# cavelandiah/BBMap

Hardware: AMD Instinct MI355X
Metric: aligned_reads_per_sec (higher is better)
Workload: dtype int32

## Files before the change

bbmap_amd/csrc/msa_common.h:

```cpp
#pragma once
#include <hip/hip_runtime.h>
#include <stdint.h>
#include "bbmap_amd.h"

namespace bbmsa {

constexpr int kScoreOffset = 11;
constexpr int kTimeMask = 0x7FF;
constexpr int kScoreMask = (int)0xFFFFF800;
constexpr int kMaxTime = 2047;

#define BBMSA_PT(x) ((x) * 2048)
constexpr int P_MATCH = BBMSA_PT(70), P_MATCH2 = BBMSA_PT(100);
constexpr int P_SUB = BBMSA_PT(-127), P_SUBR = BBMSA_PT(-147), P_SUB2 = BBMSA_PT(-51), P_SUB3 = BBMSA_PT(-25);
constexpr int P_INS = BBMSA_PT(-395), P_INS2 = BBMSA_PT(-39), P_INS3 = BBMSA_PT(-23), P_INS4 = BBMSA_PT(-8);
constexpr int P_DEL = BBMSA_PT(-472), P_DEL2 = BBMSA_PT(-33), P_DEL3 = BBMSA_PT(-9), P_DEL4 = BBMSA_PT(-1),
              P_DEL5 = BBMSA_PT(-1);
constexpr int P_DEL_REF_N = BBMSA_PT(-10), P_GAP = BBMSA_PT(-2);
constexpr int kBadOff = (-(((1 << 20) - 1) - 2000) - 1) * 2048;
constexpr int kMinOffScore = (-(((1 << 20) - 1) - 2000)) * 2048;
constexpr int kNegInf = -(1 << 30);
constexpr int kGapLen = 128;

constexpr int kTableLen = 3072;
__host__ __device__ inline int lds_table_ints(int tableLen) { return 2 * tableLen + 320; }

__host__ __device__ inline int lds_job_ints(int fastCols, int tmpBytes) { return (fastCols + 2) + ((fastCols + 2 + 3) >> 2) + ((tmpBytes + 3) >> 2); }

__host__ __device__ inline int calc_del_off(int len) {
    if (len <= 0) return 0;
    int s = P_DEL;
    if (len > 80) { s += ((len - 80 + 3) / 4) * P_DEL5; len = 80; }
    if (len > 20) { s += (len - 20) * P_DEL4; len = 20; }
    if (len > 5) { s += (len - 5) * P_DEL3; len = 5; }
    if (len > 1) s += (len - 1) * P_DEL2;
    return s;
}
__host__ __device__ inline int calc_ins_cum_off(int len) {
    if (len <= 0) return 0;
    long long s = P_INS;
    int n = len;
    if (n > 20) { s += (long long)(n - 20) * P_INS4; n = 20; }
    if (n > 5) { s += (long long)(n - 5) * P_INS3; n = 5; }
    if (n > 1) s += (long long)(n - 1) * P_INS2;
    return s < kMinOffScore ? kMinOffScore : (int)s;
}

__host__ __device__ inline bool fully_defined(int b) {
    const int u = b & ~32;
    return b < 128 && (u == 'A' || u == 'C' || u == 'G' || u == 'T' || u == 'U');
}

struct Scheme11ts {
    static constexpr int OFF = kScoreOffset, TMASK = kTimeMask, SMASK = kScoreMask, MAXT = kMaxTime;
    static constexpr int MATCH = P_MATCH, MATCH2 = P_MATCH2, SUB = P_SUB, SUBR = P_SUBR, SUB2 = P_SUB2, SUB3 = P_SUB3;
    static constexpr int INS = P_INS, INS2 = P_INS2, INS3 = P_INS3, INS4 = P_INS4;
    static constexpr int DEL = P_DEL, DEL2 = P_DEL2, DEL3 = P_DEL3, DEL4 = P_DEL4, DEL5 = P_DEL5;
    static constexpr int DEL_REF_N = P_DEL_REF_N, GAP = P_GAP;
    static constexpr int BAR_I1 = 2, BAR_D1 = 3;
    static constexpr int BADOFF = kBadOff;
    __host__ __device__ static inline int del_off(int len) { return calc_del_off(len); }
    __host__ __device__ static inline int ins_cum_off(int len) { return calc_ins_cum_off(len); }
    __host__ __device__ static inline int col0(int row) { return calc_ins_cum_off(row); }
};
struct Scheme9PacBio {
    static constexpr int OFF = 9, TMASK = 0x1FF, SMASK = (int)0xFFFFFE00, MAXT = 511;
#define BBMSA_PB(x) ((x) * 512)
    static constexpr int MATCH = BBMSA_PB(90), MATCH2 = BBMSA_PB(100);
    static constexpr int SUB = BBMSA_PB(-137), SUBR = BBMSA_PB(-157), SUB2 = BBMSA_PB(-49), SUB3 = BBMSA_PB(-25);
    static constexpr int INS = BBMSA_PB(-205), INS2 = BBMSA_PB(-42), INS3 = BBMSA_PB(-23), INS4 = BBMSA_PB(-8);
    static constexpr int DEL = BBMSA_PB(-292), DEL2 = BBMSA_PB(-37), DEL3 = BBMSA_PB(-17), DEL4 = BBMSA_PB(-2), DEL5 = BBMSA_PB(-1);
    static constexpr int DEL_REF_N = BBMSA_PB(-10), GAP = BBMSA_PB(-2);
    static constexpr int BAR_I1 = 1, BAR_D1 = 1;
    static constexpr int BADOFF = (-(((1 << 22) - 1) - 2000) - 1) * 512;
#undef BBMSA_PB
    __host__ __device__ static inline int del_off(int len) {
        if (len <= 0) return 0;
        int s = DEL;
        if (len > 80) { s += ((len - 80 + 3) / 4) * DEL5; len = 80; }
        if (len > 20) { s += (len - 20) * DEL4; len = 20; }
// ... 99 lines not shown
```

bbmap_amd/csrc/msa_fill_fast.hip:

```cpp
#include "msa_common.h"
#include "msa_cell.h"

namespace bbmsa {

__device__ __forceinline__ int lane_up(int x, int fill) {
    return __builtin_amdgcn_update_dpp(fill, x, 0x138, 0xf, 0xf, false);
}

__device__ __forceinline__ int clamp_time(int t) { return t > kMaxTime ? kMaxTime - 3 : t; }

__device__ __forceinline__ int del_extend(int streak) {
    int c = (streak & 3) == 0 ? P_DEL5 : 0;
    c = streak < 80 ? P_DEL4 : c;
    c = streak < 20 ? P_DEL3 : c;
    c = streak < 5 ? P_DEL2 : c;
    c = streak == 0 ? P_DEL : c;
    return c;
}
__device__ __forceinline__ int ins_extend(int streak) {
    int c = P_INS4;
    c = streak < 20 ? P_INS3 : c;
    c = streak < 5 ? P_INS2 : c;
    c = streak == 0 ? P_INS : c;
    return c;
}
__device__ __forceinline__ int sub_extend(int streak) {
    int c = P_SUB3;
    c = streak < 5 ? P_SUB2 : c;
    c = streak == 0 ? P_SUB : c;
    return c;
}

__device__ __forceinline__ unsigned load_coherent(const unsigned *p) {
    return __hip_atomic_load(p, __ATOMIC_RELAXED, __HIP_MEMORY_SCOPE_AGENT);
}

#ifndef BBMSA_MIN_WAVES
#define BBMSA_MIN_WAVES(R) ((R) <= 5 ? 4 : ((R) <= 7 ? 2 : 1))
#endif

template <int R, bool BANDED, bool MAT = false>
__global__ __launch_bounds__(256, BBMSA_MIN_WAVES(R)) void msa_fill_fast_kernel(const FillParams p) {
    extern __shared__ int lds[];
    int *delC = lds;
    const int TL = p.tableLen;
    int *insC = lds + TL;
    int *delExt = lds + 2 * TL;
    int *insExt = delExt + 128;
    int4 *mTab = reinterpret_cast<int4 *>(delExt + 192);
    LdsPen pen; pen.delC = delC; pen.insC = insC; pen.delExt = delExt; pen.insExt = insExt; pen.mTab = mTab;
    for (int i = threadIdx.x; i < TL; i += blockDim.x) {
        delC[i] = calc_del_off(i);
        insC[i] = calc_ins_cum_off(i);
    }
    for (int i = threadIdx.x; i < 128; i += blockDim.x) delExt[i] = del_extend(i);
    if (threadIdx.x < 32) insExt[threadIdx.x] = ins_extend(threadIdx.x);
    if (threadIdx.x < 32) {
        const int st = threadIdx.x & 7, mt = (threadIdx.x >> 3) & 1, pv = threadIdx.x >> 4;
        int4 e;
        if (mt) { e.x = pv ? P_MATCH2 : P_MATCH; e.y = P_MATCH; e.z = P_MATCH2; }
        else { e.x = pv ? (st <= 1 ? P_SUBR : P_SUB) : sub_extend(min(st, 5)); e.y = P_SUB; e.z = P_SUB3; }
        e.w = 0;
        mTab[threadIdx.x] = e;
    }
    __syncthreads();

    if (p.priority == 3) __builtin_amdgcn_s_setprio(3);
    else if (p.priority == 2) __builtin_amdgcn_s_setprio(2);
    else if (p.priority == 1) __builtin_amdgcn_s_setprio(1);
    const int lane = threadIdx.x & 63;
    const int wave = threadIdx.x >> 6;
    const int G = p.lanesPerJob;
    const int gl = lane & (G - 1);
    const int sub = lane / G;
    const int jobsPerWave = 64 / G;
    const int groupBase = sub * G;

    const int perJobLds = lds_job_ints(p.fastCols, p.tmpBytes);
    int *myLds = lds + lds_table_ints(TL) + (wave * jobsPerWave + sub) * perJobLds;
    int *colHl = myLds;
    uint8_t *colRef = reinterpret_cast<uint8_t *>(myLds + (p.fastCols + 2));
    uint8_t *tmp = reinterpret_cast<uint8_t *>(myLds + (p.fastCols + 2) + ((p.fastCols + 2 + 3) >> 2));

    const long long slot = ((long long)blockIdx.x * (blockDim.x >> 6) + wave) * jobsPerWave + sub;
    unsigned *dir = p.dirbuf + slot * p.dir_slot_dwords;

    const long long total = p.list ? (long long)load_coherent(p.list_count) : job_count(p.njobs, p.njobs_dev);
    for (;;) {
        unsigned base = 0;
        if (lane == 0) base = atomicAdd(p.queue, (unsigned)jobsPerWave);
        base = __builtin_amdgcn_readfirstlane(base);
        if ((long long)base >= total) break;
        const long long q = (long long)base + sub;
        const bool valid = q < total;
        const long long j = (p.list && valid) ? (long long)p.list[q] : q;

        bbmsa_job jb;
        if (valid) jb = p.jobs[j];
        else { jb.read_off = 0; jb.ref_off = 0; jb.read_len = 0; jb.ref_len = 0; jb.refStartLoc = 0; jb.refEndLoc = -1; jb.minScore = 0; jb.flags = 0; }
        const int rows = jb.read_len;
        int a = jb.refStartLoc, b = jb.refEndLoc;
        const int mode = jb.flags & BBMSA_MODE_MASK;
        if (jb.flags & BBMSA_CLAMP_WINDOW) {
            a = max(0, a);
            b = min(jb.ref_len - 1, b);
            if (b - a >= p.maxColumns) b = min(jb.ref_len - 1, a + p.maxColumns - 1);
        }
        const int columns = b - a + 1;
        const bool shapeOK = valid && rows >= 1 && columns >= 1 && rows <= p.maxRows && columns <= p.maxColumns;

        int halfband = 0;
        if (!(p.bandwidth < 1 && p.bandwidthRatio <= 0.0f)) {
            const int bwA = p.bandwidth < 1 ? 9999999 : p.bandwidth;
            const int bwB = p.bandwidthRatio <= 0.0f ? 9999999 : 8 + (int)__fmul_rn((float)rows, p.bandwidthRatio);
            halfband = max(min(bwA, bwB), columns - rows + 8) / 2;
        }
        int minScore = jb.minScore;
        bool limited;
        if (mode == BBMSA_FILL_UNLIMITED_RAW) limited = false;
        else if (mode == BBMSA_FILL_LIMITED_RAW) limited = true;
        else {
            if (minScore < 1 || (columns + rows < 90) ||
                ((halfband < 1 || halfband * 3 > columns) && (columns > rows + min(170, rows + 20)))) limited = false;
            else { limited = true; minScore -= 120; }
        }
        const bool fits = rows <= G * R && columns <= p.fastCols && columns >= rows - 2;
        const bool needGeneric = shapeOK && !fits;
        const bool run = shapeOK && !needGeneric;
        const bool banded = limited && halfband > 0;
        int bandViolation = 0;

        if (gl == 0 && valid) {
            if (!shapeOK) {
                bbmsa_result r;
                for (int i = 0; i < 5; i++) r.result[i] = 0;
                r.status = BBMSA_ST_BAD_SHAPE; r.iterations = 0;
                for (int i = 0; i < 8; i++) r.score[i] = 0;
                r.score_len = 0; r.match_len = 0; r.fill_kind = 0; r.columns = columns;
// ... 41 lines not shown
                cst[k] = c;
                laneSum += c;
            }
            int inc = laneSum;
            for (int d = 1; d < G; d <<= 1) {
                const int o = __shfl_down(inc, d, 64);
                if (gl + d < G) inc += o;
            }
            int suffix = inc - laneSum;
#pragma unroll
            for (int k = R - 1; k >= 0; k--) {
                suffix += cst[k];
                vlim[k] = limited ? max(minScoreOff - suffix, floorv) : kNegInf;
            }
            if (MAT && run && limited) {
                int *vout = p.limits + p.limits_off[j];
#pragma unroll
                for (int k = 0; k < R; k++) if (r0 + k < rows) vout[r0 + k] = vlim[k];
                if (gl == 0) {
                    vout[rows] = minScoreOff;
                    const int c0 = fully_defined(call1[0]) ? ((rows > 1 && fully_defined(idxByte[0])) ? P_MATCH2 : P_MATCH) : 0;
                    vout[0] = rows > 1 ? max(vlim[0] - c0, floorv) : max(minScoreOff - c0, floorv);
                }
            }
        }

        if (run) {
            for (int c = gl + 1; c <= columns; c += G) colRef[c] = rf[c - 1];
        }
        __builtin_amdgcn_fence(__ATOMIC_ACQ_REL, "wavefront");
        __builtin_amdgcn_wave_barrier();
        if (run && gl == 0) {
            int h = minScoreOff;
            bool prevDef = false;
            for (int i = columns - 1; i >= 0; i--) {
                colHl[i + 1] = (limited ? h : kNegInf) + 2048;
                const int cb = colRef[i + 1];
                const bool def = fully_defined(cb);
                const int cost = def ? (prevDef ? P_MATCH2 : P_MATCH) : ((prevDef && cb == '-') ? P_DEL : 0);
                h = max(h - cost, floorv);
                prevDef = def;
                if (MAT && limited) p.limits[p.limits_off[j] + rows + 1 + i + 1] = colHl[i + 1] - 2048;
            }
            if (MAT && limited) p.limits[p.limits_off[j] + rows + 1] = h;
        }
        __builtin_amdgcn_fence(__ATOMIC_ACQ_REL, "wavefront");
        __builtin_amdgcn_wave_barrier();

        const int nl = (rows + R - 1) / R;
        int steps = run ? columns + nl - 1 : 0;
        for (int d = 32; d >= 1; d >>= 1) steps = max(steps, __shfl_xor(steps, d, 64));

        int pM[R], pD[R], pI[R];
        int minGood[R], maxGood[R];
        int vlimP[R];
        int delForce[R];
        int insHiForce[R];
        unsigned dacc[R];
        int mPrev[R];
#pragma unroll
        for (int k = 0; k < R; k++) {
            const int row = r0 + k;
            const int c0v = insC[row];
            pM[k] = c0v; pD[k] = c0v; pI[k] = c0v;
            minGood[k] = -1; maxGood[k] = -2; dacc[k] = 0;
            vlimP[k] = rowValid[k] ? vlim[k] + 2048 : (1 << 30);
            mPrev[k] = (call1[k] == '!') ? 8 : 0;
            delForce[k] = (row < 3 || row > rows - 3) ? INT_MAX : INT_MIN;
            insHiForce[k] = (row > rows - 2) ? INT_MAX : INT_MIN;
        }
        const bool rowOne = (r0 == 1);
        const bool notLimited = !limited;
        const bool groupLead = (gl == 0);
        const int floorP = floorv + 2048;
        int svM = insC[r0 - 1], svD = svM, svI = svM;
        int lastRef = '!';
        const int lastSlot = (max(rows, 1) - 1) % R;
        const bool ownerLaneFlag = gl == (max(rows, 1) - 1) / R;
        int bestM = 0, bestD = 0, bestI = 0, bestMc = -1, bestDc = -1, bestIc = -1;

        for (int t = 1; t <= steps; t++) {
            const int c = t - gl;
            if (c >= 1 && run) {
            const bool inRange = c <= columns;
            const int cc = min(c, columns);
            const int hlP = colHl[cc], ref1 = colRef[cc];
            const int ref0 = c < 2 ? '!' : lastRef;
            const bool gap = ref1 == '-';
            const bool refN = ref1 == 'N';
            const int refPen = refN ? P_DEL_REF_N : (gap ? P_GAP : 0);
            const int insNeededBase = (columns - c) + 1;
            const bool cGt1 = c > 1;
            const int cLtLastForce = (c < columns - 1) ? INT_MAX : INT_MIN;
            const unsigned sh = (unsigned)(t & 7) * 4u;

            int upM = lane_up(pM[R - 1], 0);
            int upD = lane_up(pD[R - 1], 0);
            int upI = lane_up(pI[R - 1], 0);
            int upMin = lane_up(minGood[R - 1], 1);
            upM = groupLead ? 0 : upM; upD = groupLead ? 0 : upD; upI = groupLead ? 0 : upI;
            upMin = groupLead ? 1 : upMin;
            int upMaxG = 0;
            if (BANDED) {
                upMaxG = lane_up(maxGood[R - 1], 0);
                upMaxG = groupLead ? min(columns, 2 * halfband) : upMaxG;
            }
            int dgM = svM, dgD = svD, dgI = svI;
            svM = upM; svD = upD; svI = upI;
            bool started = upMin >= 0;
            int pm8 = ((call0First == ref0) & (ref0 != 'N')) ? 8 : 0;

#pragma unroll
            for (int k = 0; k < R; k++) {
                const int row = r0 + k;
                bool act = inRange & (started | notLimited);
                if (BANDED) act = act && (!banded || (c >= row - halfband && c <= upMaxG + 1));
                CellIn ci_;
                ci_.row = row; ci_.c = c; ci_.rows = rows; ci_.insNeededBase = insNeededBase;
                ci_.cl1 = call1[k]; ci_.ref1 = ref1; ci_.refN = refN; ci_.gap = gap; ci_.match = (call1[k] == ref1) & !refN; ci_.act = act;
                ci_.refPen = refPen; ci_.limitP = max(vlimP[k], hlP); ci_.floorP = floorP; ci_.subfloor = subfloor;
                ci_.dgM = dgM; ci_.dgD = dgD; ci_.dgI = dgI; ci_.lM = pM[k]; ci_.lD = pD[k]; ci_.upM = upM; ci_.upI = upI;
                ci_.delForce = delForce[k];
                ci_.insForce = (k == 0) ? ((rowOne && cGt1) ? INT_MAX : min(insHiForce[k], cLtLastForce)) : min(insHiForce[k], cLtLastForce);
                ci_.pm8 = pm8;
                const CellOut co = cell_update<Scheme11ts, false>(pen, ci_);
                const int nM = co.nM, nD = co.nD, nI = co.nI;
                const bool goodM = co.goodM, goodD = co.goodD, goodI = co.goodI;
                const int mb8 = co.mb8;
                if (MAT) {
                    if (inRange & rowValid[k]) {
                        int *cellp = planeM + (long long)(row - 1) * planeW + (c - 1);
                        const int sM = co.pruneM ? subfloor : (goodM ? nM : (subfloor | clamp_cell_time<Scheme11ts>(co.timeM)));
                        const int sD = co.pruneD ? subfloor : (goodD ? nD : (subfloor | clamp_cell_time<Scheme11ts>(co.timeD)));
                        const int sI = co.pruneI ? subfloor : (goodI ? nI : (subfloor | clamp_cell_time<Scheme11ts>(co.timeI)));
                        cellp[0] = sM; cellp[planeInts] = sD; cellp[2 * planeInts] = sI;
                    }
                }
                dacc[k] |= co.nib << sh;

                const bool good = goodM | goodD | goodI;
                if (BANDED) {
                    if (good && banded && minGood[k] >= 0 && c - maxGood[k] >= 3 && row < rows) bandViolation = 1;
                }
                minGood[k] = (good & (minGood[k] < 0)) ? c : minGood[k];
                maxGood[k] = good ? c : maxGood[k];
                dgM = pM[k]; dgD = pD[k]; dgI = pI[k];
                pM[k] = nM; pD[k] = nD; pI[k] = nI;
                upM = nM; upI = nI;
                started = minGood[k] >= 0;
                if (BANDED) upMaxG = maxGood[k];
                pm8 = mPrev[k];
                mPrev[k] = mb8;
            }
            lastRef = ref1;

            {
                int lm = pM[0], ld = pD[0], li = pI[0];
#pragma unroll
                for (int k = 1; k < R; k++) {
                    lm = (lastSlot == k) ? pM[k] : lm; ld = (lastSlot == k) ? pD[k] : ld; li = (lastSlot == k) ? pI[k] : li;
                }
                const bool track = ownerLaneFlag & inRange;
                const bool um = track & ((bestMc < 0) | ((lm & kScoreMask) > (bestM & kScoreMask)));
                const bool ud = track & ((bestDc < 0) | ((ld & kScoreMask) > (bestD & kScoreMask)));
                const bool ui = track & ((bestIc < 0) | ((li & kScoreMask) > (bestI & kScoreMask)));
                bestM = um ? lm : bestM; bestMc = um ? c : bestMc;
                bestD = ud ? ld : bestD; bestDc = ud ? c : bestDc;
                bestI = ui ? li : bestI; bestIc = ui ? c : bestIc;
            }
            }

            if ((t & 7) == 7) {
                const long long o = (long long)(t >> 3) * R * G + gl;
#pragma unroll
                for (int k = 0; k < R; k++) { dir[o + (long long)k * G] = dacc[k]; dacc[k] = 0; }
            }
        }
        if ((steps & 7) != 7) {
            const long long o = (long long)(steps >> 3) * R * G + gl;
#pragma unroll
            for (int k = 0; k < R; k++) dir[o + (long long)k * G] = dacc[k];
        }

        int firstNoEnter = INT_MAX;
        int lastColStart = 1, lastHasGood = 0;
        long long itersAll[R];
        {
            int pMin = lane_up(minGood[R - 1], 1), pMax = lane_up(maxGood[R - 1], columns);
            if (gl == 0) { pMin = 1; pMax = columns; }
#pragma unroll
            for (int k = 0; k < R; k++) {
                const int row = r0 + k;
                itersAll[k] = 0;
                if (rowValid[k]) {
                    const int hasGood = minGood[k] >= 0;
                    const int colStart = banded ? max(pMin, row - halfband) : pMin;
                    const int colStop = banded ? min(pMax, row + 2 * halfband - 1) : pMax;
                    const bool enter = pMin >= 0 && colStart >= 0 && colStop >= colStart;
                    if (!enter && firstNoEnter == INT_MAX) firstNoEnter = row;
                    const int endc = banded ? min(columns, colStop + 1)
                                            : min(columns, max(colStop, hasGood ? maxGood[k] : -2) + 1);
                    itersAll[k] = (long long)(endc - colStart + 1);
                    if (row == rows) { lastColStart = colStart; lastHasGood = hasGood; }
                }
                pMin = minGood[k]; pMax = maxGood[k];
            }
        }
        int groupNoEnter = firstNoEnter;
        for (int d = 1; d < G; d <<= 1) groupNoEnter = min(groupNoEnter, __shfl_xor(groupNoEnter, d, 64));
        long long iters = 0;
#pragma unroll
        for (int k = 0; k < R; k++) if (rowValid[k] && r0 + k < groupNoEnter) iters += itersAll[k];
        for (int d = 1; d < G; d <<= 1) iters += __shfl_xor(iters, d, 64);
        if (!limited) iters = (long long)rows * columns;
        for (int d = 1; d < G; d <<= 1) bandViolation |= __shfl_xor(bandViolation, d, 64);

        const int ownerLane = groupBase + (max(rows, 1) - 1) / R;
        int bScore, bCol, bState, bPacked;
        {
            int s = bestMc >= 0 ? (bestM & kScoreMask) : INT_MIN, cbest = bestMc, st = 0, pk = bestM;
            if (bestDc >= 0 && (bestD & kScoreMask) > s) { s = bestD & kScoreMask; cbest = bestDc; st = 1; pk = bestD; }
            if (bestIc >= 0 && (bestI & kScoreMask) > s) { s = bestI & kScoreMask; cbest = bestIc; st = 2; pk = bestI; }
            bScore = __shfl(s, ownerLane, 64);
            bCol = __shfl(cbest, ownerLane, 64);
            bState = __shfl(st, ownerLane, 64);
            bPacked = __shfl(pk, ownerLane, 64);
            lastColStart = __shfl(lastColStart, ownerLane, 64);
            lastHasGood = __shfl(lastHasGood, ownerLane, 64);
        }

        int res0 = rows, res1, res2, res3, res4 = 0;
        bool fillNull = false;
        if (!limited) {
            res1 = bCol; res2 = bState; res3 = bScore >> kScoreOffset;
        } else if (groupNoEnter <= rows) {
            res1 = 1; res2 = 0; res3 = kBadOff; res4 = 1; fillNull = true;
        } else if (!lastHasGood) {
            res1 = max(1, lastColStart - 1); res2 = 0; res3 = subfloor; res4 = 1; fillNull = true;
        } else if (bScore < minScoreOff) {
            res1 = bCol; res2 = bState; res3 = bScore; res4 = 1; fillNull = true;
        } else {
            res1 = bCol; res2 = bState; res3 = bScore >> kScoreOffset;
        }

        const bool wantScore = run && !fillNull && !bandViolation && (jb.flags & BBMSA_DO_SCORE);
        const bool wantTrace = run && !fillNull && !bandViolation && (jb.flags & BBMSA_DO_TRACEBACK) && p.match != nullptr;
        int sc[8] = {0, 0, 0, 0, 0, 0, 0, 0};
        int scoreLen = 0, matchLen = 0;

        asm volatile("s_waitcnt vmcnt(0)" ::: "memory");
        __builtin_amdgcn_wave_barrier();

        if (__any(wantScore || wantTrace)) {
            const bool walk = wantScore || wantTrace;
            int row = walk ? rows : 0, col = walk ? res1 : 0, state = res2;
            int n = 0, gapSyms = 0, stateTime = 0;
            while (__any(row > 0 && col > 0)) {
                const bool go = row > 0 && col > 0;
                if (go && state == 0) {
                    const int rr = row - gl, cq = col - gl;
                    const bool inside = rr >= 1 && cq >= 1;
                    unsigned nibv = 0;
                    if (inside) {
                        const int ol = (rr - 1) / R, ok = (rr - 1) - ol * R, ot = cq + ol;
                        const unsigned dw = load_coherent(dir + ((long long)(ot >> 3) * R + ok) * G + ol);
                        nibv = (dw >> ((ot & 7) * 4)) & 15u;
                    }
                    const bool brk = !inside || (nibv & 3u) != 0u;
                    unsigned long long bal = __ballot(brk);
                    unsigned long long mine = (G == 64) ? bal : ((bal >> groupBase) & ((1ull << G) - 1ull));
                    const int fb = mine ? __builtin_ctzll(mine) : G;
                    const int fbInside = __shfl((int)inside, groupBase + min(fb, G - 1), 64);
                    const int fbPrev = __shfl((int)(nibv & 3u), groupBase + min(fb, G - 1), 64);
                    const int consumed = (fb < G && fbInside) ? fb + 1 : fb;
                    if (wantTrace && gl < consumed) {
                        const int cb = rd[rr - 1], rb = colRef[cq];
                        tmp[n + gl] = (cb == rb) ? 'm' : ((!fully_defined(cb) || !fully_defined(rb)) ? 'N' : 'S');
                    }
                    stateTime += fb;
// ... 112 lines not shown
```

bbmap_amd/csrc/msa_host.hip:

```cpp
#include <hip/hip_runtime.h>

#include <cstdio>
#include <cstdlib>
#include <cstring>
#include <new>

#include "msa_common.h"

int bbmsa_align_impl(bbmsa_ctx *c, void *stream_, int64_t n_jobs, const uint32_t *n_jobs_dev, const bbmsa_job *jobs,
                     const uint8_t *reads, const uint8_t *refs, bbmsa_result *results, uint8_t *match, int32_t match_stride);

namespace bbmsa {
struct StripParams {
    const bbmsa_job *jobs; const uint8_t *reads; const uint8_t *refs; bbmsa_result *results; uint8_t *match;
    long long njobs; const unsigned int *njobs_dev; unsigned int *queue; unsigned int *dirbuf;
    long long dir_slot_dwords, dir_strip_dwords; int *boundary; uint8_t *tmpbuf; int *slow_list; unsigned int *slow_count;
    int match_stride; int maxRows, maxColumns; int bandwidth; float bandwidthRatio;
    int pipeK, pipeSlots; int *pipeBoundary; int *pipeSync; int pipeSpinLimit;
};
int strip_rows_per_lane();
const void *strip_kernel_pacbio();
const void *strip_kernel_pacbio_pipelined();
int strip_pipe_sync_ints(int K);
const void *fast_kernel_for(int R, bool banded);
// ... 18 lines not shown
    const int t = threadIdx.x;
    s[t] = hist[t];
    __syncthreads();
    for (int d = 1; d < WIDTH_BUCKETS; d <<= 1) { const unsigned v = t >= d ? s[t - d] : 0u; __syncthreads(); s[t] += v; __syncthreads(); }
    hist[t] = s[t] - hist[t];
    if (t == 0) *listCount = n;
}
__global__ void width_scatter_kernel(const bbmsa_job *jobs, long long n, int maxColumns, unsigned *cursor, int *list) {
    const long long i = (long long)blockIdx.x * blockDim.x + threadIdx.x;
    if (i < n) list[atomicAdd(&cursor[job_width_bucket(jobs[i], maxColumns)], 1u)] = (int)i;
}
}

static thread_local char g_err[512] = "";

static int fail(int code, const char *fmt, const char *detail = "") {
    snprintf(g_err, sizeof g_err, fmt, detail);
    return code;
}
#define HIP_TRY(expr)                                                                      \
    do {                                                                                   \
        hipError_t e_ = (expr);                                                            \
        if (e_ != hipSuccess) {                                                            \
            snprintf(g_err, sizeof g_err, "%s failed: %s", #expr, hipGetErrorString(e_));  \
            return BBMAP_E_HIP;                                                            \
        }                                                                                  \
    } while (0)

#include "msa_ctx.h"

extern "C" const char *bbmap_last_error(void) { return g_err; }
void bbmap_set_error(const char *msg) { snprintf(g_err, sizeof g_err, "%s", msg); }
extern "C" int bbmap_abi_version(void) { return BBMAP_AMD_ABI_VERSION; }

static int env_int(const char *name, int dflt) {
    const char *v = getenv(name);
    return (v && *v) ? atoi(v) : dflt;
}

static int setup_wide_pass(bbmsa_ctx *c) {
    if (c->wideBlocks > 0) return BBMAP_OK;
    c->wideR = (c->cfg.maxRows + 63) / 64;
    c->wideCols = c->cfg.maxColumns;
    c->wideTmpBytes = ((64 * c->wideR + c->wideCols + 8) + 3) & ~3;
    const int perJob = bbmsa::lds_job_ints(c->wideCols, c->wideTmpBytes);
    c->wideLdsBytes = (bbmsa::lds_table_ints(c->wideTableLen) + perJob) * 4;
    const void *wfn = bbmsa::fast_kernel_for(c->wideR, c->banded);
    if (wfn && c->wideLdsBytes <= 160 * 1024) {
        if (c->wideLdsBytes > 64 * 1024) HIP_TRY(hipFuncSetAttribute(wfn, hipFuncAttributeMaxDynamicSharedMemorySize, c->wideLdsBytes));
        int per = 0;
        HIP_TRY(hipOccupancyMaxActiveBlocksPerMultiprocessor(&per, wfn, 64, c->wideLdsBytes));
        if (per < 1) per = 1;
        if (per > 8) per = 8;
        const long long slotDwords = (long long)(((c->wideCols + 64 - 1) >> 3) + 1) * c->wideR * 64;
        HIP_TRY(hipMalloc(&c->d_wideDir, (size_t)((long long)c->numCUs * per * slotDwords * 4)));
        c->wideDirSlotDwords = slotDwords;
        c->wideBlocks = c->numCUs * per;
    }
    return BBMAP_OK;
}

extern "C" int bbmsa_create(const bbmsa_config *cfg, bbmsa_ctx **out) {
    if (!cfg || !out) return fail(BBMAP_E_ARG, "bbmsa_create: null argument");
    *out = nullptr;
    const int scheme = cfg->reserved[2] & 0xFF;
    const bool legacyOnly = (cfg->reserved[2] & BBMSA_LEGACY_ONLY) != 0;
    if (scheme != BBMSA_SCHEME_11TS && scheme != BBMSA_SCHEME_9PACBIO) return fail(BBMAP_E_ARG, "bbmsa_create: unknown scoring scheme");
    if (scheme == BBMSA_SCHEME_11TS && (cfg->maxRows < 1 || cfg->maxRows > 640 || cfg->maxColumns < 1 || cfg->maxColumns > 4096))
        return fail(BBMAP_E_ARG, "bbmsa_create: maxRows must be 1..640 and maxColumns 1..4096");
    if (scheme == BBMSA_SCHEME_9PACBIO && (cfg->maxRows < 1 || cfg->maxRows > 6100 || cfg->maxColumns < 1 || cfg->maxColumns > 8192))
        return fail(BBMAP_E_ARG, "bbmsa_create: the PacBio scheme takes maxRows 1..6100 and maxColumns 1..8192");
    int ndev = 0;
    if (hipGetDeviceCount(&ndev) != hipSuccess || ndev <= 0)
        return fail(BBMAP_E_NODEVICE, "bbmsa_create: no HIP device (this library has no CPU path)");
    if (cfg->device < 0 || cfg->device >= ndev) return fail(BBMAP_E_ARG, "bbmsa_create: bad device ordinal");
    HIP_TRY(hipSetDevice(cfg->device));
    hipDeviceProp_t prop;
    HIP_TRY(hipGetDeviceProperties(&prop, cfg->device));
    if (strncmp(prop.gcnArchName, "gfx950", 6) != 0)
        return fail(BBMAP_E_NODEVICE, "bbmsa_create: device is %s, this build targets gfx950 only", prop.gcnArchName);

    bbmsa_ctx *c = new (std::nothrow) bbmsa_ctx();
    if (!c) return fail(BBMAP_E_NOMEM, "bbmsa_create: out of host memory");
    memset(c, 0, sizeof *c);
    c->cfg = *cfg;
    c->device = cfg->device;
    c->numCUs = prop.multiProcessorCount;

    c->scheme = scheme;
    c->legacyOnly = legacyOnly;
    struct Guard { bbmsa_ctx *c; ~Guard() { if (c) bbmsa_destroy(c); } } guard{c};
    if (legacyOnly) {
        HIP_TRY(hipMalloc(&c->d_counters, 64));
        HIP_TRY(hipMemset(c->d_counters, 0, 64));
        const long long planeInts = (long long)(cfg->maxRows + 1) * (cfg->maxColumns + 2);
        c->genThreads = 1;
        HIP_TRY(hipMalloc(&c->d_matrix, (size_t)(3 * planeInts * 4)));
        HIP_TRY(hipMalloc(&c->d_limits, (size_t)((cfg->maxRows + cfg->maxColumns + 4) * 4)));
        for (int i = 0; i < 4; i++) HIP_TRY(hipEventCreate(&c->ev[i]));
        { const int rc = bbmsa_legacy_create(c); if (rc != BBMAP_OK) return rc; }
        guard.c = nullptr;
        *out = c;
        return BBMAP_OK;
    }
    if (scheme != BBMSA_SCHEME_11TS) {
        HIP_TRY(hipMalloc(&c->d_counters, 64));
        HIP_TRY(hipMemset(c->d_counters, 0, 64));
// ... 37 lines not shown
                if (c->pipeJobsMax > 0) {
                    HIP_TRY(hipMalloc(&c->d_pipeBoundary, (size_t)((long long)c->pipeSlots * strips * 3 * (cfg->maxColumns + 2) * 4)));
                    HIP_TRY(hipMalloc(&c->d_pipeSync, (size_t)((long long)c->pipeSlots * bbmsa::strip_pipe_sync_ints(strips) * 4)));
                }
            }
            HIP_TRY(hipMalloc(&c->d_dir, (size_t)((long long)c->stripBlocks * c->stripSlotDwords * 4)));
            HIP_TRY(hipMalloc(&c->d_stripBoundary, (size_t)((long long)c->stripBlocks * 6 * (cfg->maxColumns + 2) * 4)));
            HIP_TRY(hipMalloc(&c->d_stripTmp, (size_t)((long long)c->stripBlocks * (cfg->maxRows + cfg->maxColumns + 8))));
        }
        for (int i = 0; i < 4; i++) HIP_TRY(hipEventCreate(&c->ev[i]));
        guard.c = nullptr;
        *out = c;
        return BBMAP_OK;
    }
    int G = cfg->reserved[0];
    if (G != 16 && G != 32 && G != 64) {
        G = env_int("BBMSA_LANES_PER_JOB", 0);
        if (G != 16 && G != 32 && G != 64) G = (cfg->maxRows <= 320) ? 32 : 64;
    }
    while (G < 64 && (cfg->maxRows + G - 1) / G > 10) G *= 2;
    c->G = G;
    c->R = (cfg->maxRows + G - 1) / G;
    int fastCols = cfg->reserved[1] > 0 ? cfg->reserved[1] : env_int("BBMSA_FAST_COLS", 0);
    if (fastCols <= 0) fastCols = cfg->maxColumns < 640 ? cfg->maxColumns : 640;
    if (fastCols > cfg->maxColumns) fastCols = cfg->maxColumns;
    c->fastCols = fastCols;
    c->tmpBytes = ((G * c->R + fastCols + 8) + 3) & ~3;
    const int jobsPerWave = 64 / G;
    const int perJobInts = bbmsa::lds_job_ints(fastCols, c->tmpBytes);
    {
        const int side = (cfg->maxColumns > cfg->maxRows ? cfg->maxColumns : cfg->maxRows) + 2;
        c->wideTableLen = (side < 2048 ? side : 2048) + cfg->maxRows + 8;
        const int sideF = (fastCols > cfg->maxRows ? fastCols : cfg->maxRows) + 2;
        c->tableLen = (sideF < 2048 ? sideF : 2048) + cfg->maxRows + 8;
    }
    if (c->tableLen > bbmsa::kTableLen) c->tableLen = bbmsa::kTableLen;
    if (c->wideTableLen > bbmsa::kTableLen) c->wideTableLen = bbmsa::kTableLen;
    c->tableLen = (c->tableLen + 3) & ~3; c->wideTableLen = (c->wideTableLen + 3) & ~3;
    c->ldsBytes = (bbmsa::lds_table_ints(c->tableLen) + 4 * jobsPerWave * perJobInts) * 4;
    if (c->ldsBytes > 160 * 1024) return fail(BBMAP_E_ARG, "bbmsa_create: fast-path LDS budget exceeded; lower reserved[1] (fastCols)");

    c->banded = !(cfg->bandwidth < 1 && cfg->bandwidthRatio <= 0.0f);
    const void *kfn = bbmsa::fast_kernel_for(c->R, c->banded);
    if (!kfn) return fail(BBMAP_E_ARG, "bbmsa_create: no kernel for this rows-per-lane");
    if (c->ldsBytes > 64 * 1024)
        HIP_TRY(hipFuncSetAttribute(kfn, hipFuncAttributeMaxDynamicSharedMemorySize, c->ldsBytes));
    int blocksPerCU = 0;
    HIP_TRY(hipOccupancyMaxActiveBlocksPerMultiprocessor(&blocksPerCU, kfn, 256, c->ldsBytes));
    if (blocksPerCU < 1) blocksPerCU = 1;
    const int capBlocks = env_int("BBMSA_BLOCKS_PER_CU", 0);
    if (capBlocks > 0 && capBlocks < blocksPerCU) blocksPerCU = capBlocks;
    c->blocks = c->numCUs * blocksPerCU;

    const int maxSteps = fastCols + G - 1;
    c->dirSlotDwords = (long long)((maxSteps >> 3) + 1) * c->R * G;
    const long long slots = (long long)c->blocks * 4 * jobsPerWave;
    HIP_TRY(hipMalloc(&c->d_dir, (size_t)(slots * c->dirSlotDwords * 4)));
    HIP_TRY(hipMalloc(&c->d_counters, 64));
    HIP_TRY(hipMemset(c->d_counters, 0, 64));

    const long long planeInts = (long long)(cfg->maxRows + 1) * (cfg->maxColumns + 2);
    const long long perThread = 3 * planeInts * 4;
    long long budget = (long long)env_int("BBMSA_GENERIC_SCRATCH_MB", 2048) << 20;
    long long threads = budget / perThread;
    if (threads > 16384) threads = 16384;
    threads = (threads / 64) * 64;
    if (threads < 64) return fail(BBMAP_E_NOMEM, "bbmsa_create: BBMSA_GENERIC_SCRATCH_MB cannot hold one wavefront of scratch matrices for this maxRows x maxColumns");
    c->genThreads = (int)threads;
    HIP_TRY(hipMalloc(&c->d_matrix, (size_t)(threads * perThread)));
    HIP_TRY(hipMalloc(&c->d_limits, (size_t)(threads * (cfg->maxRows + cfg->maxColumns + 4) * 4)));
    c->wideBlocks = 0; c->latencyJobs = 0;
    if (cfg->maxColumns > fastCols) { const int rc = setup_wide_pass(c); if (rc != BBMAP_OK) return rc; }
    c->narrowBlocks = 0; c->narrowOff = false; c->narrowUsed = false;
    c->sortByWidth = false; c->d_widthHist = nullptr;
    c->narrowSlack = env_int("BBMSA_NARROW_SLACK", 2000);
    if (!c->banded && env_int("BBMSA_NARROW", 1) != 0) {
        int perCU = 0;
        HIP_TRY(hipOccupancyMaxActiveBlocksPerMultiprocessor(&perCU, (const void *)bbmsa::msa_fill_narrow_kernel, 64, 0));
        if (perCU < 1) perCU = 1;
        if (perCU > 16) perCU = 16;
        c->narrowBlocks = c->numCUs * perCU;
        HIP_TRY(hipMalloc(&c->d_narrowDir, (size_t)c->narrowBlocks * (size_t)(cfg->maxRows + 1) * 64 * 8));
    }
    for (int i = 0; i < 4; i++) HIP_TRY(hipEventCreate(&c->ev[i]));
    guard.c = nullptr;
    *out = c;
    return BBMAP_OK;
}

extern "C" void bbmsa_destroy(bbmsa_ctx *c) {
    if (!c) return;
    (void)hipSetDevice(c->device);
    bbmsa_legacy_destroy(c);
    if (c->d_dir) (void)hipFree(c->d_dir);
    if (c->d_counters) (void)hipFree(c->d_counters);
    if (c->d_widthHist) (void)hipFree(c->d_widthHist);

    if (c->d_slowList) (void)hipFree(c->d_slowList);
    if (c->d_matrix) (void)hipFree(c->d_matrix);
    if (c->d_limits) (void)hipFree(c->d_limits);
    if (c->d_wideDir) (void)hipFree(c->d_wideDir);
    if (c->d_slowList2) (void)hipFree(c->d_slowList2);
    if (c->d_narrowDir) (void)hipFree(c->d_narrowDir);
    if (c->d_fastList) (void)hipFree(c->d_fastList);
    if (c->d_gref) (void)hipFree(c->d_gref);
    if (c->d_gaux) (void)hipFree(c->d_gaux);
    if (c->d_gjobs) (void)hipFree(c->d_gjobs);
    if (c->d_stripBoundary) (void)hipFree(c->d_stripBoundary);
// ... 253 lines not shown
```

bbmap_amd/csrc/msa_legacy.hip:

```cpp
#include <hip/hip_runtime.h>

#include <chrono>
#include <condition_variable>
#include <cstdio>
#include <cstdlib>
#include <cstring>
#include <mutex>
#include <new>

#include "msa_common.h"
#include "msa_ctx.h"

void bbmap_set_error(const char *msg);

namespace bbmsa {
const void *fast_kernel_mat_for(int R, bool banded);
template <class S> __global__ void msa_fill_generic_kernel(const GenericParams p);
}

namespace {

int lfail(int code, const char *msg) { bbmap_set_error(msg); return code; }
#define L_TRY(expr)                                                                               \
    do {                                                                                          \
// ... 201 lines not shown
    S->leaderActive = false;
    S->cv.notify_all();
}

}

int bbmsa_legacy_create(bbmsa_ctx *c) {
    bbmsa_legacy *S = new (std::nothrow) bbmsa_legacy();
    if (!S) return lfail(BBMAP_E_NOMEM, "bbmsa_create: out of host memory");
    c->legacy = S;
    S->open = 0; S->leaderActive = false; S->nextGen = 1; S->calls = S->launches = S->handed = 0; S->nsWave = S->nsHanded = S->nsWaitReaders = 0;
    S->stream = nullptr; S->d_dir = nullptr;
    memset(S->B, 0, sizeof S->B);
    const int maxRows = c->cfg.maxRows, maxCols = c->cfg.maxColumns;
    const long long oneJobInts = 3LL * maxRows * maxCols;
    long long poolInts = ((long long)env_int("BBMSA_LEGACY_POOL_MB", 64) << 20) / 4;
    if (poolInts < oneJobInts) poolInts = oneJobInts;
    S->capInts = poolInts;
    S->capJobs = env_int("BBMSA_LEGACY_BATCH", 1024);
    if (S->capJobs < 1) S->capJobs = 1;
    S->capBytes = (long long)S->capJobs * 1024;
    if (S->capBytes < maxRows + maxCols + 16) S->capBytes = maxRows + maxCols + 16;
    S->capLimits = (long long)S->capJobs * 512;
    if (S->capLimits < maxRows + maxCols + 8) S->capLimits = maxRows + maxCols + 8;
    S->offPlaneOff = (long long)S->capJobs * sizeof(bbmsa_job);
    S->offLimitsOff = S->offPlaneOff + (long long)S->capJobs * 8;
    S->offBytes = S->offLimitsOff + (long long)S->capJobs * 8;
    L_TRY(hipStreamCreateWithFlags(&S->stream, hipStreamNonBlocking));
    for (int i = 0; i < 2; i++) { const int rc = alloc_batch(S, S->B[i]); if (rc != BBMAP_OK) return rc; }
    S->B[0].gen = S->nextGen;
    S->wave = false;
    if (c->scheme == BBMSA_SCHEME_11TS) {
        S->R = (maxRows + 63) / 64;
        S->cols = maxCols;
        S->tmpBytes = ((64 * S->R + S->cols + 8) + 3) & ~3;
        const int side = (maxCols > maxRows ? maxCols : maxRows) + 2;
        S->tableLen = (side < 2048 ? side : 2048) + maxRows + 8;
        if (S->tableLen > bbmsa::kTableLen) S->tableLen = bbmsa::kTableLen;
        S->tableLen = (S->tableLen + 3) & ~3;
        const int perJob = bbmsa::lds_job_ints(S->cols, S->tmpBytes);
        S->ldsBytes = (bbmsa::lds_table_ints(S->tableLen) + perJob) * 4;
        c->banded = !(c->cfg.bandwidth < 1 && c->cfg.bandwidthRatio <= 0.0f);
        const void *kfn = bbmsa::fast_kernel_mat_for(S->R, c->banded);
        if (kfn && S->ldsBytes <= 160 * 1024) {
            if (S->ldsBytes > 64 * 1024)
                for (int r = 1; r <= S->R; r++)
                    L_TRY(hipFuncSetAttribute(bbmsa::fast_kernel_mat_for(r, c->banded), hipFuncAttributeMaxDynamicSharedMemorySize, S->ldsBytes));
            int per = 0;
            L_TRY(hipOccupancyMaxActiveBlocksPerMultiprocessor(&per, kfn, 64, S->ldsBytes));
            if (per < 1) per = 1;
            if (per > 8) per = 8;
            S->blocks = c->numCUs * per;
            if (S->blocks > S->capJobs) S->blocks = S->capJobs;
            S->dirSlotDwords = (long long)(((S->cols + 64 - 1) >> 3) + 1) * S->R * 64;
            L_TRY(hipMalloc((void **)&S->d_dir, (size_t)((long long)S->blocks * S->dirSlotDwords * 4)));
            S->wave = true;
        }
    }
    return BBMAP_OK;
}

void bbmsa_legacy_destroy(bbmsa_ctx *c) {
    bbmsa_legacy *S = c->legacy;
    if (!S) return;
    if (S->stream) { (void)hipStreamSynchronize(S->stream); (void)hipStreamDestroy(S->stream); }
    for (int i = 0; i < 2; i++) free_batch(S->B[i]);
    if (S->d_dir) (void)hipFree(S->d_dir);
    delete S;
    c->legacy = nullptr;
}

extern "C" int bbmsa_fill_submit(bbmsa_ctx *c, const uint8_t *read, int32_t read_len, const uint8_t *ref, int32_t ref_len,
                                 int32_t refStartLoc, int32_t refEndLoc, int32_t minScore, int32_t mode,
                                 int32_t *result5, int64_t *iterations, bbmsa_ticket *ticket) {
    if (!c || !read || !ref || !result5 || !ticket) return lfail(BBMAP_E_ARG, "bbmsa_fill_submit: null argument");
    if (!c->legacy) return lfail(BBMAP_E_ARG, "bbmsa_fill_submit: the context was not created with BBMSA_LEGACY_ONLY");
    if (mode != BBMSA_FILL_LIMITED_RAW && mode != BBMSA_FILL_UNLIMITED_RAW) return lfail(BBMAP_E_ARG, "bbmsa_fill_submit: mode must be one of the two raw fills");
    const int rows = read_len;
    const long long columns = (long long)refEndLoc - refStartLoc + 1;
    if (rows < 1 || columns < 1 || rows > c->cfg.maxRows || columns > c->cfg.maxColumns || refStartLoc < 0 || refEndLoc >= ref_len)
        return lfail(BBMAP_E_SHAPE, "bbmsa_fill_submit: problem exceeds the context limits or its reference array");
    bbmsa_legacy *S = c->legacy;
    const long long needBytes = ((long long)rows + columns + 7) & ~7LL;
    const long long needInts = 3LL * rows * columns;
    const long long needLimits = rows + columns + 2;
    std::unique_lock<std::mutex> lk(S->mu);
    S->calls++;
    Batch *b;
    for (;;) {
        b = &S->B[S->open];
        if (b->njobs < S->capJobs && b->usedBytes + needBytes <= S->capBytes && b->usedInts + needInts <= S->capInts &&
            b->usedLimits + needLimits <= S->capLimits) break;
        if (!S->leaderActive) { S->leaderActive = true; lead(c, lk); }
        else S->cv.wait(lk);
    }
    const int slot = b->njobs++;
    const long long myGen = b->gen;
    uint8_t *bytes = b->h_in + S->offBytes + b->usedBytes;
    memcpy(bytes, read, (size_t)rows);
    memcpy(bytes + rows, ref + refStartLoc, (size_t)columns);
    bbmsa_job &jb = b->jobs()[slot];
    jb.read_off = b->usedBytes; jb.ref_off = b->usedBytes + rows; jb.read_len = rows; jb.ref_len = (int32_t)columns;
    jb.refStartLoc = 0; jb.refEndLoc = (int32_t)columns - 1; jb.minScore = minScore; jb.flags = mode;
    ((long long *)(b->h_in + S->offPlaneOff))[slot] = b->usedInts;
    ((long long *)(b->h_in + S->offLimitsOff))[slot] = b->usedLimits;
    b->usedBytes += needBytes; b->usedInts += needInts; b->usedLimits += needLimits;
    while (!(b->state == DONE && b->gen == myGen)) {
// ... 63 lines not shown
```

Baseline: 9.057 million.

## Pack per-row good-column range into u16x2 and defer last-row best search

Replaces the separate minGood/maxGood registers with one packed u16x2 word updated by a packed max. The last row's M/D/I values are now written to a per-slot global buffer each step, instead of being compared and tracked in six best-score registers, and a wave-parallel reduction afterwards finds the best column. The aim is to cut VGPR pressure and per-step ALU work in the inner DP loop. In exchange it adds a global store on every step, a larger dir slot allocation, and a reduction pass after the fill.

```diff
diff --git a/bbmap_amd/csrc/msa_common.h b/bbmap_amd/csrc/msa_common.h
--- a/bbmap_amd/csrc/msa_common.h
+++ b/bbmap_amd/csrc/msa_common.h
@@ -26,6 +26,9 @@
 __host__ __device__ inline int lds_table_ints(int tableLen) { return 2 * tableLen + 320; }
 
 __host__ __device__ inline int lds_job_ints(int fastCols, int tmpBytes) { return (fastCols + 2) + ((fastCols + 2 + 3) >> 2) + ((tmpBytes + 3) >> 2); }
+
+__host__ __device__ inline long long fast_dir_record_dwords(int cols, int G, int R) { return (long long)(((cols + G - 1) >> 3) + 1) * R * G; }
+__host__ __device__ inline long long fast_dir_slot_dwords(int cols, int G, int R) { return (fast_dir_record_dwords(cols, G, R) + 3LL * (cols + 1) + 63) & ~63LL; }
 
 __host__ __device__ inline int calc_del_off(int len) {
     if (len <= 0) return 0;
diff --git a/bbmap_amd/csrc/msa_fill_fast.hip b/bbmap_amd/csrc/msa_fill_fast.hip
--- a/bbmap_amd/csrc/msa_fill_fast.hip
+++ b/bbmap_amd/csrc/msa_fill_fast.hip
@@ -6,6 +6,13 @@
 __device__ __forceinline__ int lane_up(int x, int fill) {
     return __builtin_amdgcn_update_dpp(fill, x, 0x138, 0xf, 0xf, false);
 }
+
+__device__ __forceinline__ unsigned pk_max_u16(unsigned a, unsigned b) {
+    typedef unsigned short u16x2 __attribute__((ext_vector_type(2)));
+    return __builtin_bit_cast(unsigned, __builtin_elementwise_max(__builtin_bit_cast(u16x2, a), __builtin_bit_cast(u16x2, b)));
+}
+__device__ __forceinline__ int ext_first(unsigned e) { return (e & 0xffffu) ? 0xffff - (int)(e & 0xffffu) : -1; }
+__device__ __forceinline__ int ext_last(unsigned e) { return (int)(e >> 16) - 2; }
 
 __device__ __forceinline__ int clamp_time(int t) { return t > kMaxTime ? kMaxTime - 3 : t; }
 
@@ -84,6 +91,7 @@
 
     const long long slot = ((long long)blockIdx.x * (blockDim.x >> 6) + wave) * jobsPerWave + sub;
     unsigned *dir = p.dirbuf + slot * p.dir_slot_dwords;
+    unsigned *lastRow = dir + fast_dir_record_dwords(p.fastCols, G, R);
 
     const long long total = p.list ? (long long)load_coherent(p.list_count) : job_count(p.njobs, p.njobs_dev);
     for (;;) {
@@ -231,7 +239,7 @@
         for (int d = 32; d >= 1; d >>= 1) steps = max(steps, __shfl_xor(steps, d, 64));
 
         int pM[R], pD[R], pI[R];
-        int minGood[R], maxGood[R];
+        unsigned goodExt[R];
         int vlimP[R];
         int delForce[R];
         int insHiForce[R];
@@ -242,7 +250,7 @@
             const int row = r0 + k;
             const int c0v = insC[row];
             pM[k] = c0v; pD[k] = c0v; pI[k] = c0v;
-            minGood[k] = -1; maxGood[k] = -2; dacc[k] = 0;
+            goodExt[k] = 0u; dacc[k] = 0;
             vlimP[k] = rowValid[k] ? vlim[k] + 2048 : (1 << 30);
             mPrev[k] = (call1[k] == '!') ? 8 : 0;
             delForce[k] = (row < 3 || row > rows - 3) ? INT_MAX : INT_MIN;
@@ -256,7 +264,6 @@
         int lastRef = '!';
         const int lastSlot = (max(rows, 1) - 1) % R;
         const bool ownerLaneFlag = gl == (max(rows, 1) - 1) / R;
-        int bestM = 0, bestD = 0, bestI = 0, bestMc = -1, bestDc = -1, bestIc = -1;
 
         for (int t = 1; t <= steps; t++) {
             const int c = t - gl;
@@ -272,21 +279,22 @@
             const bool cGt1 = c > 1;
             const int cLtLastForce = (c < columns - 1) ? INT_MAX : INT_MIN;
             const unsigned sh = (unsigned)(t & 7) * 4u;
+            const unsigned cExt = ((unsigned)(c + 2) << 16) | (unsigned)(0xffff - c);
 
             int upM = lane_up(pM[R - 1], 0);
             int upD = lane_up(pD[R - 1], 0);
             int upI = lane_up(pI[R - 1], 0);
-            int upMin = lane_up(minGood[R - 1], 1);
+            int upExt = lane_up((int)goodExt[R - 1], 1);
             upM = groupLead ? 0 : upM; upD = groupLead ? 0 : upD; upI = groupLead ? 0 : upI;
-            upMin = groupLead ? 1 : upMin;
+            upExt = groupLead ? 1 : upExt;
             int upMaxG = 0;
             if (BANDED) {
-                upMaxG = lane_up(maxGood[R - 1], 0);
+                upMaxG = ((unsigned)upExt >> 16) - 2;
                 upMaxG = groupLead ? min(columns, 2 * halfband) : upMaxG;
             }
             int dgM = svM, dgD = svD, dgI = svI;
             svM = upM; svD = upD; svI = upI;
-            bool started = upMin >= 0;
+            bool started = upExt != 0;
             int pm8 = ((call0First == ref0) & (ref0 != 'N')) ? 8 : 0;
 
 #pragma unroll
@@ -319,15 +327,14 @@
 
                 const bool good = goodM | goodD | goodI;
                 if (BANDED) {
-                    if (good && banded && minGood[k] >= 0 && c - maxGood[k] >= 3 && row < rows) bandViolation = 1;
-                }
-                minGood[k] = (good & (minGood[k] < 0)) ? c : minGood[k];
-                maxGood[k] = good ? c : maxGood[k];
+                    if (good && banded && goodExt[k] != 0u && c - (int)(goodExt[k] >> 16) + 2 >= 3 && row < rows) bandViolation = 1;
+                }
+                goodExt[k] = good ? pk_max_u16(goodExt[k], cExt) : goodExt[k];
                 dgM = pM[k]; dgD = pD[k]; dgI = pI[k];
                 pM[k] = nM; pD[k] = nD; pI[k] = nI;
                 upM = nM; upI = nI;
-                started = minGood[k] >= 0;
-                if (BANDED) upMaxG = maxGood[k];
+                started = goodExt[k] != 0u;
+                if (BANDED) upMaxG = (int)(goodExt[k] >> 16) - 2;
                 pm8 = mPrev[k];
                 mPrev[k] = mb8;
             }
@@ -339,13 +346,8 @@
                 for (int k = 1; k < R; k++) {
                     lm = (lastSlot == k) ? pM[k] : lm; ld = (lastSlot == k) ? pD[k] : ld; li = (lastSlot == k) ? pI[k] : li;
                 }
-                const bool track = ownerLaneFlag & inRange;
-                const bool um = track & ((bestMc < 0) | ((lm & kScoreMask) > (bestM & kScoreMask)));
-                const bool ud = track & ((bestDc < 0) | ((ld & kScoreMask) > (bestD & kScoreMask)));
-                const bool ui = track & ((bestIc < 0) | ((li & kScoreMask) > (bestI & kScoreMask)));
-                bestM = um ? lm : bestM; bestMc = um ? c : bestMc;
-                bestD = ud ? ld : bestD; bestDc = ud ? c : bestDc;
-                bestI = ui ? li : bestI; bestIc = ui ? c : bestIc;
+                unsigned *lr = lastRow + ((ownerLaneFlag & inRange) ? 3 * c : 0);
+                lr[0] = (unsigned)lm; lr[1] = (unsigned)ld; lr[2] = (unsigned)li;
             }
             }
 
@@ -365,24 +367,25 @@
         int lastColStart = 1, lastHasGood = 0;
         long long itersAll[R];
         {
-            int pMin = lane_up(minGood[R - 1], 1), pMax = lane_up(maxGood[R - 1], columns);
+            const unsigned upE = (unsigned)lane_up((int)goodExt[R - 1], 0);
+            int pMin = ext_first(upE), pMax = ext_last(upE);
             if (gl == 0) { pMin = 1; pMax = columns; }
 #pragma unroll
             for (int k = 0; k < R; k++) {
                 const int row = r0 + k;
                 itersAll[k] = 0;
                 if (rowValid[k]) {
-                    const int hasGood = minGood[k] >= 0;
+                    const int hasGood = goodExt[k] != 0u;
                     const int colStart = banded ? max(pMin, row - halfband) : pMin;
                     const int colStop = banded ? min(pMax, row + 2 * halfband - 1) : pMax;
                     const bool enter = pMin >= 0 && colStart >= 0 && colStop >= colStart;
                     if (!enter && firstNoEnter == INT_MAX) firstNoEnter = row;
                     const int endc = banded ? min(columns, colStop + 1)
-                                            : min(columns, max(colStop, hasGood ? maxGood[k] : -2) + 1);
+                                            : min(columns, max(colStop, hasGood ? ext_last(goodExt[k]) : -2) + 1);
                     itersAll[k] = (long long)(endc - colStart + 1);
                     if (row == rows) { lastColStart = colStart; lastHasGood = hasGood; }
                 }
-                pMin = minGood[k]; pMax = maxGood[k];
+                pMin = ext_first(goodExt[k]); pMax = ext_last(goodExt[k]);
             }
         }
         int groupNoEnter = firstNoEnter;
@@ -397,13 +400,30 @@
         const int ownerLane = groupBase + (max(rows, 1) - 1) / R;
         int bScore, bCol, bState, bPacked;
         {
-            int s = bestMc >= 0 ? (bestM & kScoreMask) : INT_MIN, cbest = bestMc, st = 0, pk = bestM;
-            if (bestDc >= 0 && (bestD & kScoreMask) > s) { s = bestD & kScoreMask; cbest = bestDc; st = 1; pk = bestD; }
-            if (bestIc >= 0 && (bestI & kScoreMask) > s) { s = bestI & kScoreMask; cbest = bestIc; st = 2; pk = bestI; }
-            bScore = __shfl(s, ownerLane, 64);
-            bCol = __shfl(cbest, ownerLane, 64);
-            bState = __shfl(st, ownerLane, 64);
-            bPacked = __shfl(pk, ownerLane, 64);
+            asm volatile("s_waitcnt vmcnt(0)" ::: "memory");
+            __builtin_amdgcn_wave_barrier();
+            int sP[3] = {INT_MIN, INT_MIN, INT_MIN}, cP[3] = {-1, -1, -1};
+            const int lastCol = run ? columns : 0;
+            for (int cq = gl + 1; cq <= lastCol; cq += G) {
+#pragma unroll
+                for (int q = 0; q < 3; q++) {
+                    const int v = (int)load_coherent(lastRow + 3 * cq + q) & kScoreMask;
+                    if (cP[q] < 0 || v > sP[q]) { sP[q] = v; cP[q] = cq; }
+                }
+            }
+#pragma unroll
+            for (int q = 0; q < 3; q++) {
+                for (int d = 1; d < G; d <<= 1) {
+                    const int so = __shfl_xor(sP[q], d, 64), co = __shfl_xor(cP[q], d, 64);
+                    const bool take = co >= 0 && (cP[q] < 0 || so > sP[q] || (so == sP[q] && co < cP[q]));
+                    sP[q] = take ? so : sP[q]; cP[q] = take ? co : cP[q];
+                }
+            }
+            int s = cP[0] >= 0 ? sP[0] : INT_MIN, cbest = cP[0], st = 0;
+            if (cP[1] >= 0 && sP[1] > s) { s = sP[1]; cbest = cP[1]; st = 1; }
+            if (cP[2] >= 0 && sP[2] > s) { s = sP[2]; cbest = cP[2]; st = 2; }
+            bScore = s; bCol = cbest; bState = st;
+            bPacked = cbest >= 0 ? (int)load_coherent(lastRow + 3 * cbest + st) : 0;
             lastColStart = __shfl(lastColStart, ownerLane, 64);
             lastHasGood = __shfl(lastHasGood, ownerLane, 64);
         }
diff --git a/bbmap_amd/csrc/msa_host.hip b/bbmap_amd/csrc/msa_host.hip
--- a/bbmap_amd/csrc/msa_host.hip
+++ b/bbmap_amd/csrc/msa_host.hip
@@ -94,7 +94,7 @@
         HIP_TRY(hipOccupancyMaxActiveBlocksPerMultiprocessor(&per, wfn, 64, c->wideLdsBytes));
         if (per < 1) per = 1;
         if (per > 8) per = 8;
-        const long long slotDwords = (long long)(((c->wideCols + 64 - 1) >> 3) + 1) * c->wideR * 64;
+        const long long slotDwords = bbmsa::fast_dir_slot_dwords(c->wideCols, 64, c->wideR);
         HIP_TRY(hipMalloc(&c->d_wideDir, (size_t)((long long)c->numCUs * per * slotDwords * 4)));
         c->wideDirSlotDwords = slotDwords;
         c->wideBlocks = c->numCUs * per;
@@ -238,8 +238,7 @@
     if (capBlocks > 0 && capBlocks < blocksPerCU) blocksPerCU = capBlocks;
     c->blocks = c->numCUs * blocksPerCU;
 
-    const int maxSteps = fastCols + G - 1;
-    c->dirSlotDwords = (long long)((maxSteps >> 3) + 1) * c->R * G;
+    c->dirSlotDwords = bbmsa::fast_dir_slot_dwords(fastCols, G, c->R);
     const long long slots = (long long)c->blocks * 4 * jobsPerWave;
     HIP_TRY(hipMalloc(&c->d_dir, (size_t)(slots * c->dirSlotDwords * 4)));
     HIP_TRY(hipMalloc(&c->d_counters, 64));
diff --git a/bbmap_amd/csrc/msa_legacy.hip b/bbmap_amd/csrc/msa_legacy.hip
--- a/bbmap_amd/csrc/msa_legacy.hip
+++ b/bbmap_amd/csrc/msa_legacy.hip
@@ -277,7 +277,7 @@
             if (per > 8) per = 8;
             S->blocks = c->numCUs * per;
             if (S->blocks > S->capJobs) S->blocks = S->capJobs;
-            S->dirSlotDwords = (long long)(((S->cols + 64 - 1) >> 3) + 1) * S->R * 64;
+            S->dirSlotDwords = bbmsa::fast_dir_slot_dwords(S->cols, 64, S->R);
             L_TRY(hipMalloc((void **)&S->d_dir, (size_t)((long long)S->blocks * S->dirSlotDwords * 4)));
             S->wave = true;
         }
```

Result: no change. 9.141 million, median of 6 (+0.9%).
